# VITA-Group/UVC

Hardware: AMD Instinct MI355X
Metric: images/sec UVC Stage-1 step, DeiT-Tiny budget=0.5 (higher is better)
Workload: dtype bf16; 1 GPU; deit_tiny_patch16_224 Stage-1 UVC-train step, budget 0.5, per-GPU batch 512, 224x224x3 synthetic, soft distillation alpha 0.1, block gating on; global_batch=512, parallelism=dp1

## Files before the change

### uvc_amd/csrc/gemm_nt_ws.hip

```cpp
#include "gemm_common.h"

constexpr int WS_BM = 64;

template <typename TA, typename TC, int EPI, int KT, int WS_NW, int NJ = 4>
__global__ __launch_bounds__(64 * WS_NW, (KT > 6 && WS_NW > 6) ? 1 : (NJ == 4 || KT > 6) ? 2 : 4) void k_gemm_ws(NtArgs g, int ngroups, int nslots) {
  typedef bf16_t T;
  typedef Mma<T> MM;
  constexpr int ROWB = KT * 64 + 32;
  constexpr int CPR = KT * 4;
  constexpr int NLD = (WS_BM * CPR + 64 * WS_NW - 1) / (64 * WS_NW);
  constexpr int CW = 16 * NJ, EPW = CW + 4;
  constexpr int VN = OutVec<TC>::VN, LPR = CW / VN, RPI = 64 / LPR;
  constexpr bool DYN = KT > 6;
  constexpr int IMGB = WS_BM * ROWB;
  extern __shared__ __attribute__((aligned(16))) char ws_dyn[];
  __shared__ __attribute__((aligned(16))) char sA_st[DYN ? 16 : 2 * IMGB];
  __shared__ __attribute__((aligned(16))) float sStage_st[DYN ? 4 : WS_NW * 16 * EPW];
  char* const sAb = DYN ? ws_dyn : sA_st;
  float* const sStg = DYN ? reinterpret_cast<float*>(ws_dyn + 2 * IMGB) : sStage_st;
  const int tid = threadIdx.x, lane = tid & 63, w = tid >> 6, gq = lane >> 4, li = lane & 15;
  const int L = blockIdx.x;
  const int grp = (L >> 3) % ngroups, slot = (L / (8 * ngroups)) * 8 + (L & 7);
  const int n0 = grp * CW * WS_NW + w * CW;
  const bool active = n0 < g.N;
  const TA* __restrict__ A = reinterpret_cast<const TA*>(g.A);
  const T* __restrict__ W = reinterpret_cast<const T*>(g.B);
  TC* __restrict__ C = reinterpret_cast<TC*>(g.C);
  const int ntiles = (g.M + WS_BM - 1) / WS_BM;

  typename MM::Frag bf[NJ][KT];
  if (active) {
#pragma unroll
    for (int j = 0; j < NJ; ++j)
#pragma unroll
      for (int ks = 0; ks < KT; ++ks)
        bf[j][ks] = __builtin_bit_cast(typename MM::Frag, *reinterpret_cast<const u32x4*>(W + (size_t)(n0 + j * 16 + li) * g.ldb + (ks * 4 + gq) * 8));
  }
  float alpha = g.alpha;
  if (g.alpha_ptr) alpha *= *g.alpha_ptr;
  float d0 = 0.f, d1 = 1.f;
  if (EPI == UVC_EPI_BIAS_RESID_GATE) { d0 = g.dptr[0]; d1 = g.dptr[1]; }
  const int cc = (lane % LPR) * VN;
  const int n = n0 + cc;
  float bias_v[VN];
#pragma unroll
  for (int e = 0; e < VN; ++e) bias_v[e] = 0.f;
  if (active && (EPI == UVC_EPI_BIAS || EPI == UVC_EPI_BIAS_GELU || EPI == UVC_EPI_BIAS_GELU_OUT || EPI == UVC_EPI_BIAS_RESID || EPI == UVC_EPI_BIAS_RESID_GATE ||
                 EPI == UVC_EPI_BIAS_GELU_GRAD || EPI == UVC_EPI_BIAS_GELU_GRAD_Q8)) {
#pragma unroll
    for (int e = 0; e < VN; ++e) bias_v[e] = g.bias[n + e];
  }

  u32x4 ra[NLD];
  auto gload = [&](int tile) {
    const int m0 = tile * WS_BM;
    const u32x4 z = {0u, 0u, 0u, 0u};
#pragma unroll
    for (int i = 0; i < NLD; ++i) {
      const int id = tid + 64 * WS_NW * i, row = id / CPR, c = id % CPR;
      const int m = m0 + row;
      ra[i] = (row < WS_BM && m < g.M) ? ChunkLoad<TA, T>::ld(A + (size_t)m * g.lda + c * 8) : z;
    }
  };
  auto lstore = [&](int buf) {
#pragma unroll
    for (int i = 0; i < NLD; ++i) {
      const int id = tid + 64 * WS_NW * i, row = id / CPR, c = id % CPR;
      if (row < WS_BM) *reinterpret_cast<u32x4*>(sAb + buf * IMGB + row * ROWB + c * 16) = ra[i];
    }
  };

  constexpr int IT = 16 / RPI;
  struct Epi { u32x4 r[IT]; u32x4 r2[IT]; u32x4 ax[IT]; };
  auto eload = [&](Epi& E, int tile_, int sub_) {
    if (!active) return;
#pragma unroll
    for (int it = 0; it < IT; ++it) {
      const int m = tile_ * WS_BM + sub_ * 16 + it * RPI + lane / LPR;
      const bool ok = m < g.M && tile_ < ntiles;
      const size_t mo = (size_t)(ok ? m : 0);
      if (EPI == UVC_EPI_BIAS_RESID || EPI == UVC_EPI_BIAS_RESID_GATE) E.r[it] = *reinterpret_cast<const u32x4*>(reinterpret_cast<const TC*>(g.R) + mo * g.ldr + n);
      if (EPI == UVC_EPI_BIAS_RESID_GATE) E.r2[it] = *reinterpret_cast<const u32x4*>(reinterpret_cast<const TC*>(g.R2) + mo * g.ldr + n);
      if (EPI == UVC_EPI_DGELU || EPI == UVC_EPI_MUL_AUX) {
        if constexpr (VN == 8) E.ax[it] = *reinterpret_cast<const u32x4*>(reinterpret_cast<const T*>(g.aux) + mo * g.ldaux + n);
        else {
          const u32x2 q = *reinterpret_cast<const u32x2*>(reinterpret_cast<const T*>(g.aux) + mo * g.ldaux + n);
          E.ax[it][0] = q[0]; E.ax[it][1] = q[1];
        }
      }
      if (EPI == UVC_EPI_MUL_AUX_Q8) {
        const u32x2 q = *reinterpret_cast<const u32x2*>(reinterpret_cast<const unsigned char*>(g.aux) + mo * g.ldaux + n);
        E.ax[it][0] = q[0]; E.ax[it][1] = q[1];
      }
    }
  };
  auto subtile = [&](int buf_, int m0_, int sub_, const Epi& E) {
    if (!active) return;
    float* stg = sStg + w * (16 * EPW);
    {
      typename MM::Frag fa[KT];
#pragma unroll
      for (int ks = 0; ks < KT; ++ks) fa[ks] = lds_frag<T>(sAb + buf_ * IMGB + (sub_ * 16 + li) * ROWB + (ks * 4 + gq) * 16);
#pragma unroll
      for (int j = 0; j < NJ; ++j) {
        f32x4 c = {0.f, 0.f, 0.f, 0.f};
#pragma unroll
        for (int ks = 0; ks < KT; ++ks) c = MM::mma(bf[j][ks], fa[ks], c);
        *reinterpret_cast<f32x4*>(stg + li * EPW + j * 16 + gq * 4) = c;
      }
    }
    __builtin_amdgcn_wave_barrier();
    unsigned qc[IT][2];
#pragma unroll
    for (int it = 0; it < IT; ++it) { qc[it][0] = 0u; qc[it][1] = 0u; }
#pragma unroll
    for (int it = 0; it < IT; ++it) {
      const int r = it * RPI + lane / LPR;
      const int m = m0_ + sub_ * 16 + r;
      float v[VN];
      load_vec<float, VN>(stg + r * EPW + cc, v);
      if (m < g.M) {
        const size_t mo = (size_t)m;
#pragma unroll
        for (int e = 0; e < VN; ++e) v[e] = epi_scale_bias(v[e], alpha, bias_v[e]);
        if (EPI == UVC_EPI_BIAS_RESID || EPI == UVC_EPI_BIAS_RESID_GATE) {
          float rv[VN];
          Resid<TC>::get(E.r[it], rv);
#pragma unroll
          for (int e = 0; e < VN; ++e) v[e] += rv[e];
        }
        if (EPI == UVC_EPI_BIAS_RESID_GATE) {
          float rv[VN];
          Resid<TC>::get(E.r2[it], rv);
#pragma unroll
          for (int e = 0; e < VN; ++e) v[e] = epi_gate_mix(v[e], rv[e], d0, d1);
        }
        if (EPI == UVC_EPI_DGELU) {
#pragma unroll
          for (int e = 0; e < VN / 2; ++e) {
            v[2 * e] *= Gelu<T>::g(__uint_as_float(E.ax[it][e] << 16));
            v[2 * e + 1] *= Gelu<T>::g(__uint_as_float(E.ax[it][e] & 0xffff0000u));
          }
        }
        if (EPI == UVC_EPI_MUL_AUX) {
#pragma unroll
          for (int e = 0; e < VN / 2; ++e) {
            v[2 * e] *= __uint_as_float(E.ax[it][e] << 16);
            v[2 * e + 1] *= __uint_as_float(E.ax[it][e] & 0xffff0000u);
          }
        }
        if constexpr (EPI == UVC_EPI_MUL_AUX_Q8) {
          static_assert(VN == 8, "q8 epilogue: bf16 C");
#pragma unroll
          for (int e = 0; e < 8; ++e)
            v[e] *= __builtin_fmaf((float)((E.ax[it][e >> 2] >> (8 * (e & 3))) & 0xffu), UVC_Q8_STEP, UVC_Q8_LO);
        }
        if (EPI == UVC_EPI_BIAS_GELU_OUT) {
#pragma unroll
          for (int e = 0; e < VN; ++e) v[e] = Gelu<T>::f(v[e]);
        }
        float u[VN];
        if (EPI == UVC_EPI_BIAS_GELU_GRAD || EPI == UVC_EPI_BIAS_GELU_GRAD_Q8) {
#pragma unroll
          for (int e = 0; e < VN; ++e) { float fo, go; Gelu<T>::fg(v[e], fo, go); u[e] = fo; v[e] = go; }
        }
        if constexpr (EPI == UVC_EPI_BIAS_GELU_GRAD_Q8) {
          static_assert(VN == 8, "q8 epilogue: bf16 C2");
          unsigned qw[2] = {0u, 0u};
#pragma unroll
          for (int e = 0; e < 8; ++e)
            qw[e >> 2] = __builtin_amdgcn_cvt_pk_u8_f32(__builtin_fmaf(v[e], 1.0f / UVC_Q8_STEP, -UVC_Q8_LO / UVC_Q8_STEP), e & 3, qw[e >> 2]);
          qc[it][0] = qw[0]; qc[it][1] = qw[1];
          OutVec<TC>::st_nt(reinterpret_cast<TC*>(g.C2) + mo * g.ldc + n, u);
        } else {
        if constexpr (EPI == UVC_EPI_BIAS_GELU_GRAD && sizeof(TC) == 2 && KT == 6) OutVec<TC>::st_nt(C + mo * g.ldc + n, v);
        else
        OutVec<TC>::st(C + mo * g.ldc + n, v);
        if (EPI == UVC_EPI_BIAS_GELU || EPI == UVC_EPI_BIAS_GELU_GRAD) {
          if (EPI == UVC_EPI_BIAS_GELU) {
#pragma unroll
            for (int e = 0; e < VN; ++e) u[e] = Gelu<T>::f(v[e]);
          }
          if constexpr (EPI == UVC_EPI_BIAS_GELU_GRAD && sizeof(TC) == 2 && KT == 6) OutVec<TC>::st_nt(reinterpret_cast<TC*>(g.C2) + mo * g.ldc + n, u);
          else
          OutVec<TC>::st(reinterpret_cast<TC*>(g.C2) + mo * g.ldc + n, u);
        }
        }
      }
    }
    if constexpr (EPI == UVC_EPI_BIAS_GELU_GRAD_Q8) {
      const bool odd = lane & 1;
      if constexpr (IT == 2) {
        static_assert(LPR == 8 && RPI == 8, "q8 epilogue: four waves x 64 columns");
        const unsigned s0 = odd ? qc[0][0] : qc[1][0], s1 = odd ? qc[0][1] : qc[1][1];
        const unsigned r0 = (unsigned)__builtin_amdgcn_mov_dpp((int)s0, 0xB1, 0xF, 0xF, true);
        const unsigned r1 = (unsigned)__builtin_amdgcn_mov_dpp((int)s1, 0xB1, 0xF, 0xF, true);
        const int m = m0_ + sub_ * 16 + (odd ? RPI : 0) + lane / LPR;
        if (m < g.M) {
          const u32x4 o = odd ? u32x4{r0, r1, qc[1][0], qc[1][1]} : u32x4{qc[0][0], qc[0][1], r0, r1};
          __builtin_nontemporal_store(o, reinterpret_cast<u32x4*>(reinterpret_cast<unsigned char*>(g.C) + (size_t)m * g.ldc + (n & ~15)));
        }
      } else {
        static_assert(IT == 1 && LPR == 4, "q8 epilogue: eight waves x 32 columns");
        const unsigned r0 = (unsigned)__builtin_amdgcn_mov_dpp((int)qc[0][0], 0xB1, 0xF, 0xF, true);
        const unsigned r1 = (unsigned)__builtin_amdgcn_mov_dpp((int)qc[0][1], 0xB1, 0xF, 0xF, true);
        const int m = m0_ + sub_ * 16 + lane / LPR;
        if (m < g.M && !odd)
          __builtin_nontemporal_store(u32x4{qc[0][0], qc[0][1], r0, r1}, reinterpret_cast<u32x4*>(reinterpret_cast<unsigned char*>(g.C) + (size_t)m * g.ldc + n));
      }
    }
    __builtin_amdgcn_wave_barrier();
  };

  int tile = slot;
  if (tile >= ntiles) return;
  Epi E0, E1;
  gload(tile);
  eload(E0, tile, 0);
  lstore(0);
  __syncthreads();
  int buf = 0;
  for (; tile < ntiles; tile += nslots) {
    const int next = tile + nslots;
    if (next < ntiles) gload(next);
    const int m0 = tile * WS_BM;
    eload(E1, tile, 1);
    subtile(buf, m0, 0, E0);
    eload(E0, tile, 2);
    subtile(buf, m0, 1, E1);
    eload(E1, tile, 3);
    subtile(buf, m0, 2, E0);
    eload(E0, next, 0);
    subtile(buf, m0, 3, E1);
    if (next < ntiles) lstore(buf ^ 1);
    __syncthreads();
    buf ^= 1;
  }
}

namespace {

int ws_slots(const NtArgs& a, int ngroups, int wgs) {
  const int ntiles = ceil_div(a.M, WS_BM);
  int nslots = (wgs / ngroups) & ~7;
  if (nslots < 8) nslots = 8;
  if (nslots > ((ntiles + 7) & ~7)) nslots = (ntiles + 7) & ~7;
  return nslots;
}
template <typename TA, typename TC, int KT, int WS_NW>
int launch_ws_epi(const NtArgs& a, int epi, hipStream_t st) {
  const int ngroups = ceil_div(a.N, 64 * WS_NW), nslots = ws_slots(a, ngroups, 512);
  const int grid = nslots * ngroups;
  if (epi == UVC_EPI_BIAS_GELU_GRAD_Q8) {
    if constexpr (sizeof(TA) == 2 && sizeof(TC) == 2 && KT == 6 && WS_NW == 4) {
      k_gemm_ws<TA, TC, UVC_EPI_BIAS_GELU_GRAD_Q8, KT, WS_NW><<<grid, 64 * WS_NW, 0, st>>>(a, ngroups, nslots);
      UVC_CHECK_LAUNCH();
      return UVC_OK;
    } else return uvc_set_error_msg(UVC_ERR_UNSUPPORTED, "uvc_gemm_nt: UVC_EPI_BIAS_GELU_GRAD_Q8 outside uvc_gemm_nt_q8_supported");
  }
#define WS_CASE(E) case E: k_gemm_ws<TA, TC, E, KT, WS_NW><<<grid, 64 * WS_NW, 0, st>>>(a, ngroups, nslots); break;
  NT_LAUNCH(epi, NT_EPI9(WS_CASE))
#undef WS_CASE
}
template <typename TA, typename TC, int KT>
int launch_ws_narrow(const NtArgs& a, int epi, hipStream_t st) {
  const int ngroups = ceil_div(a.N, 256), nslots = ws_slots(a, ngroups, 512);
  const int grid = nslots * ngroups;
#define WS_CASE(E) case E: k_gemm_ws<TA, TC, E, KT, 8, 2><<<grid, 512, 0, st>>>(a, ngroups, nslots); break;
  NT_LAUNCH(epi, WS_CASE(UVC_EPI_DGELU) WS_CASE(UVC_EPI_MUL_AUX) WS_CASE(UVC_EPI_MUL_AUX_Q8) WS_CASE(UVC_EPI_BIAS_GELU_GRAD_Q8))
#undef WS_CASE
}
template <typename TA, typename TC>
int launch_ws_t(const uvc_gemm_route& r, const NtArgs& a, hipStream_t st) {
  if constexpr (sizeof(TC) == 2 && sizeof(TA) == 2) {
    if (r.nw == 8) return launch_ws_narrow<TA, TC, 6>(a, r.epilogue, st);
  }
  if (r.kt == 6) return r.nw == 4 ? launch_ws_epi<TA, TC, 6, 4>(a, r.epilogue, st) : launch_ws_epi<TA, TC, 6, 3>(a, r.epilogue, st);
  return r.nw == 4 ? launch_ws_epi<TA, TC, 4, 4>(a, r.epilogue, st) : launch_ws_epi<TA, TC, 4, 3>(a, r.epilogue, st);
}
template <typename TC, int NW = 6>
int launch_ws384_t(const NtArgs& a, int epi, hipStream_t st) {
  constexpr int KT = 12, NJ = 2;
  const int ngroups = ceil_div(a.N, 32 * NW), nslots = ws_slots(a, ngroups, 256);
  const int grid = nslots * ngroups;
  const int sh = 2 * WS_BM * (KT * 64 + 32) + NW * 16 * (16 * NJ + 4) * 4;
#define WS_CASE(E) case E: { \
    UVC_MAX_LDS(sh, k_gemm_ws<bf16_t, TC, E, KT, NW, NJ>); \
    k_gemm_ws<bf16_t, TC, E, KT, NW, NJ><<<grid, 64 * NW, sh, st>>>(a, ngroups, nslots); } break;
  NT_LAUNCH(epi, WS_CASE(UVC_EPI_NONE) WS_CASE(UVC_EPI_BIAS) WS_CASE(UVC_EPI_BIAS_GELU) WS_CASE(UVC_EPI_BIAS_RESID) WS_CASE(UVC_EPI_BIAS_RESID_GATE)
                      WS_CASE(UVC_EPI_BIAS_GELU_OUT) WS_CASE(UVC_EPI_BIAS_GELU_GRAD) WS_CASE(UVC_EPI_MUL_AUX))
#undef WS_CASE
}

}

namespace uvc_gemm {
int launch_ws(const uvc_gemm_route& r, const NtArgs& a, hipStream_t st) { return NT_BY_TA_TC(launch_ws_t, r, a, st); }
int launch_ws384(const uvc_gemm_route& r, const NtArgs& a, hipStream_t st) {
  return r.nw == 8 ? launch_ws384_t<bf16_t, 8>(a, r.epilogue, st) : NT_BY_TC(launch_ws384_t, a, r.epilogue, st);
}
}
```

Measured before the change: 48340 images/sec.

## Restructure weight-stationary GEMM loop with edge specialization and deeper epilogue prefetch

Rewrites the main tile loop of the weight-stationary NT GEMM as a lambda walk, specialized at compile time on whether the wave is active and whether the tile is a full or an edge tile. Full tiles skip the per-row M bounds checks. Global loads clamp the row index instead of zero-filling. For residual, gate and aux-multiply epilogues, loads are prefetched two sub-tiles ahead through a four-deep buffer. Scheduling barriers, readfirstlane on the wave index and empty asm register pins are added to steer instruction ordering and register allocation, at the cost of more register pressure and larger code.

```diff
diff --git a/uvc_amd/csrc/gemm_nt_ws.hip b/uvc_amd/csrc/gemm_nt_ws.hip
--- a/uvc_amd/csrc/gemm_nt_ws.hip
+++ b/uvc_amd/csrc/gemm_nt_ws.hip
@@ -18,7 +18,8 @@
   __shared__ __attribute__((aligned(16))) float sStage_st[DYN ? 4 : WS_NW * 16 * EPW];
   char* const sAb = DYN ? ws_dyn : sA_st;
   float* const sStg = DYN ? reinterpret_cast<float*>(ws_dyn + 2 * IMGB) : sStage_st;
-  const int tid = threadIdx.x, lane = tid & 63, w = tid >> 6, gq = lane >> 4, li = lane & 15;
+  int tid = threadIdx.x, lane = tid & 63, gq = lane >> 4, li = lane & 15;
+  const int w = __builtin_amdgcn_readfirstlane(tid >> 6);
   const int L = blockIdx.x;
   const int grp = (L >> 3) % ngroups, slot = (L / (8 * ngroups)) * 8 + (L & 7);
   const int n0 = grp * CW * WS_NW + w * CW;
@@ -40,8 +41,8 @@
   if (g.alpha_ptr) alpha *= *g.alpha_ptr;
   float d0 = 0.f, d1 = 1.f;
   if (EPI == UVC_EPI_BIAS_RESID_GATE) { d0 = g.dptr[0]; d1 = g.dptr[1]; }
-  const int cc = (lane % LPR) * VN;
-  const int n = n0 + cc;
+  int cc = (lane % LPR) * VN;
+  int n = n0 + cc;
   float bias_v[VN];
 #pragma unroll
   for (int e = 0; e < VN; ++e) bias_v[e] = 0.f;
@@ -53,27 +54,26 @@
 
   u32x4 ra[NLD];
   auto gload = [&](int tile) {
-    const int m0 = tile * WS_BM;
-    const u32x4 z = {0u, 0u, 0u, 0u};
+    const int m0 = (tile < ntiles ? tile : ntiles - 1) * WS_BM;
 #pragma unroll
     for (int i = 0; i < NLD; ++i) {
       const int id = tid + 64 * WS_NW * i, row = id / CPR, c = id % CPR;
       const int m = m0 + row;
-      ra[i] = (row < WS_BM && m < g.M) ? ChunkLoad<TA, T>::ld(A + (size_t)m * g.lda + c * 8) : z;
+      ra[i] = ChunkLoad<TA, T>::ld(A + (size_t)(m < g.M ? m : g.M - 1) * g.lda + c * 8);
+      if constexpr (sizeof(TA) == 4) { if (i & 1) asm volatile("" : "+v"(ra[i - 1]), "+v"(ra[i]) :: "memory"); }
     }
   };
   auto lstore = [&](int buf) {
 #pragma unroll
     for (int i = 0; i < NLD; ++i) {
       const int id = tid + 64 * WS_NW * i, row = id / CPR, c = id % CPR;
-      if (row < WS_BM) *reinterpret_cast<u32x4*>(sAb + buf * IMGB + row * ROWB + c * 16) = ra[i];
+      if (WS_BM * CPR == NLD * 64 * WS_NW || row < WS_BM) *reinterpret_cast<u32x4*>(sAb + buf * IMGB + row * ROWB + c * 16) = ra[i];
     }
   };
 
   constexpr int IT = 16 / RPI;
   struct Epi { u32x4 r[IT]; u32x4 r2[IT]; u32x4 ax[IT]; };
   auto eload = [&](Epi& E, int tile_, int sub_) {
-    if (!active) return;
 #pragma unroll
     for (int it = 0; it < IT; ++it) {
       const int m = tile_ * WS_BM + sub_ * 16 + it * RPI + lane / LPR;
@@ -94,8 +94,8 @@
       }
     }
   };
-  auto subtile = [&](int buf_, int m0_, int sub_, const Epi& E) {
-    if (!active) return;
+  auto subtile = [&](auto edge_, int buf_, int m0_, int sub_, const Epi& E) {
+    constexpr bool EDGE = decltype(edge_)::value;
     float* stg = sStg + w * (16 * EPW);
     {
       typename MM::Frag fa[KT];
@@ -110,6 +110,7 @@
       }
     }
     __builtin_amdgcn_wave_barrier();
+    __builtin_amdgcn_sched_barrier(0);
     unsigned qc[IT][2];
 #pragma unroll
     for (int it = 0; it < IT; ++it) { qc[it][0] = 0u; qc[it][1] = 0u; }
@@ -119,7 +120,7 @@
       const int m = m0_ + sub_ * 16 + r;
       float v[VN];
       load_vec<float, VN>(stg + r * EPW + cc, v);
-      if (m < g.M) {
+      if (!EDGE || m < g.M) {
         const size_t mo = (size_t)m;
 #pragma unroll
         for (int e = 0; e < VN; ++e) v[e] = epi_scale_bias(v[e], alpha, bias_v[e]);
@@ -196,7 +197,7 @@
         const unsigned r0 = (unsigned)__builtin_amdgcn_mov_dpp((int)s0, 0xB1, 0xF, 0xF, true);
         const unsigned r1 = (unsigned)__builtin_amdgcn_mov_dpp((int)s1, 0xB1, 0xF, 0xF, true);
         const int m = m0_ + sub_ * 16 + (odd ? RPI : 0) + lane / LPR;
-        if (m < g.M) {
+        if (!EDGE || m < g.M) {
           const u32x4 o = odd ? u32x4{r0, r1, qc[1][0], qc[1][1]} : u32x4{qc[0][0], qc[0][1], r0, r1};
           __builtin_nontemporal_store(o, reinterpret_cast<u32x4*>(reinterpret_cast<unsigned char*>(g.C) + (size_t)m * g.ldc + (n & ~15)));
         }
@@ -205,37 +206,66 @@
         const unsigned r0 = (unsigned)__builtin_amdgcn_mov_dpp((int)qc[0][0], 0xB1, 0xF, 0xF, true);
         const unsigned r1 = (unsigned)__builtin_amdgcn_mov_dpp((int)qc[0][1], 0xB1, 0xF, 0xF, true);
         const int m = m0_ + sub_ * 16 + lane / LPR;
-        if (m < g.M && !odd)
+        if ((!EDGE || m < g.M) && !odd)
           __builtin_nontemporal_store(u32x4{qc[0][0], qc[0][1], r0, r1}, reinterpret_cast<u32x4*>(reinterpret_cast<unsigned char*>(g.C) + (size_t)m * g.ldc + n));
       }
     }
     __builtin_amdgcn_wave_barrier();
   };
 
-  int tile = slot;
-  if (tile >= ntiles) return;
-  Epi E0, E1;
-  gload(tile);
-  eload(E0, tile, 0);
-  lstore(0);
-  __syncthreads();
-  int buf = 0;
-  for (; tile < ntiles; tile += nslots) {
-    const int next = tile + nslots;
-    if (next < ntiles) gload(next);
-    const int m0 = tile * WS_BM;
-    eload(E1, tile, 1);
-    subtile(buf, m0, 0, E0);
-    eload(E0, tile, 2);
-    subtile(buf, m0, 1, E1);
-    eload(E1, tile, 3);
-    subtile(buf, m0, 2, E0);
-    eload(E0, next, 0);
-    subtile(buf, m0, 3, E1);
-    if (next < ntiles) lstore(buf ^ 1);
+  const int slot0 = slot;
+  if (slot0 >= ntiles) return;
+  const int nfull = g.M / WS_BM;
+  constexpr bool PRE2 = EPI == UVC_EPI_MUL_AUX_Q8 || EPI == UVC_EPI_MUL_AUX || (EPI == UVC_EPI_DGELU && NJ == 2) ||
+                        ((EPI == UVC_EPI_BIAS_RESID || EPI == UVC_EPI_BIAS_RESID_GATE) && sizeof(TC) == 2);
+  constexpr int EPD = PRE2 ? 2 : 1;
+  auto walk = [&](auto act_) {
+    constexpr bool ACT = decltype(act_)::value;
+    int tile = slot0, buf = 0;
+    Epi E[4];
+    if constexpr (ACT) {
+#pragma unroll
+      for (int k = 0; k < EPD; ++k) eload(E[k], tile, k);
+    }
+    gload(tile);
+    lstore(0);
+    if constexpr (ACT) {
+#pragma unroll
+      for (int k = 0; k < EPD; ++k)
+#pragma unroll
+        for (int it = 0; it < IT; ++it) {
+          if (EPI == UVC_EPI_BIAS_RESID || EPI == UVC_EPI_BIAS_RESID_GATE) asm volatile("" : "+v"(E[k].r[it]));
+          if (EPI == UVC_EPI_BIAS_RESID_GATE) asm volatile("" : "+v"(E[k].r2[it]));
+          if (EPI == UVC_EPI_DGELU || EPI == UVC_EPI_MUL_AUX) { if constexpr (VN == 8) asm volatile("" : "+v"(E[k].ax[it])); else asm volatile("" : "+v"(E[k].ax[it][0]), "+v"(E[k].ax[it][1])); }
+          if (EPI == UVC_EPI_MUL_AUX_Q8) asm volatile("" : "+v"(E[k].ax[it][0]), "+v"(E[k].ax[it][1]));
+        }
+    }
     __syncthreads();
-    buf ^= 1;
-  }
+    auto body = [&](auto edge_) {
+      const int next = tile + nslots, m0 = tile * WS_BM;
+      asm volatile("" : "+v"(tid), "+v"(lane), "+v"(gq), "+v"(li), "+v"(cc), "+v"(n));
+      gload(next);
+      if constexpr (ACT) {
+#pragma unroll
+        for (int sub = 0; sub < 4; ++sub) {
+          const int k = sub + EPD;
+          if (k < 4) eload(E[k & 3], tile, k); else eload(E[k & 3], next, k - 4);
+          subtile(edge_, buf, m0, sub, E[sub]);
+          __builtin_amdgcn_sched_barrier(0);
+        }
+      }
+      lstore(buf ^ 1);
+      __syncthreads();
+      buf ^= 1;
+    };
+    if constexpr (sizeof(TA) == 4 || (EPI == UVC_EPI_BIAS_RESID_GATE && sizeof(TC) == 4)) {
+      for (; tile < ntiles; tile += nslots) body(std::true_type{});
+    } else {
+      for (; tile < nfull; tile += nslots) body(std::false_type{});
+      if (tile < ntiles) body(std::true_type{});
+    }
+  };
+  if (active) walk(std::true_type{}); else walk(std::false_type{});
 }
 
 namespace {
```

Measured after the change: 48800 images/sec, median of 6. No clear change (+1.0%).
